# lucidrains/magvit2-pytorch

Hardware: NVIDIA H100
Metric: video-frames/sec tokenize+decode, 17x128x128 bf16 (higher is better)
Workload: dtype bf16

## Files before the change

### magvit2_pytorch_b200/csrc/tc_common.cuh

```cuda
#pragma once
#include "common.cuh"
#include <cuda.h>
#include <mutex>

namespace mv2 {


__device__ __forceinline__ uint32_t smem_u32(const void* p) { return (uint32_t)__cvta_generic_to_shared(p); }

__device__ __forceinline__ void mbar_init(uint32_t bar, uint32_t count) {
  asm volatile("mbarrier.init.shared::cta.b64 [%0], %1;" ::"r"(bar), "r"(count));
}
__device__ __forceinline__ void mbar_expect_tx(uint32_t bar, uint32_t bytes) {
  asm volatile("mbarrier.arrive.expect_tx.shared::cta.b64 _, [%0], %1;" ::"r"(bar), "r"(bytes) : "memory");
}
__device__ __forceinline__ void mbar_wait(uint32_t bar, uint32_t parity) {
  asm volatile(
      "{\n\t"
      ".reg .pred P1;\n\t"
      "WAIT_LOOP:\n\t"
      "mbarrier.try_wait.parity.shared::cta.b64 P1, [%0], %1, 0x989680;\n\t"
      "@P1 bra DONE;\n\t"
      "bra WAIT_LOOP;\n\t"
      "DONE:\n\t"
      "}" ::"r"(bar), "r"(parity) : "memory");
}
__device__ __forceinline__ void fence_barrier_init() { asm volatile("fence.mbarrier_init.release.cluster;" ::: "memory"); }
__device__ __forceinline__ void fence_proxy_async() { asm volatile("fence.proxy.async.shared::cta;" ::: "memory"); }

__device__ __forceinline__ void tma_load_5d(uint32_t dst, const CUtensorMap* map, uint32_t bar, int c0, int c1, int c2,
                                            int c3, int c4) {
  asm volatile(
      "cp.async.bulk.tensor.5d.shared::cluster.global.tile.mbarrier::complete_tx::bytes [%0], [%1, {%3, %4, %5, %6, %7}], [%2];"
      ::"r"(dst), "l"(map), "r"(bar), "r"(c0), "r"(c1), "r"(c2), "r"(c3), "r"(c4) : "memory");
}
__device__ __forceinline__ void tma_load_2d(uint32_t dst, const CUtensorMap* map, uint32_t bar, int c0, int c1) {
  asm volatile(
      "cp.async.bulk.tensor.2d.shared::cluster.global.tile.mbarrier::complete_tx::bytes [%0], [%1, {%3, %4}], [%2];"
      ::"r"(dst), "l"(map), "r"(bar), "r"(c0), "r"(c1) : "memory");
}
__device__ __forceinline__ void tma_load_3d(uint32_t dst, const CUtensorMap* map, uint32_t bar, int c0, int c1, int c2) {
  asm volatile(
      "cp.async.bulk.tensor.3d.shared::cluster.global.tile.mbarrier::complete_tx::bytes [%0], [%1, {%3, %4, %5}], [%2];"
      ::"r"(dst), "l"(map), "r"(bar), "r"(c0), "r"(c1), "r"(c2) : "memory");
}
__device__ __forceinline__ void tma_prefetch_desc(const CUtensorMap* map) {
  asm volatile("prefetch.tensormap [%0];" ::"l"(map) : "memory");
}

__device__ __forceinline__ void wgmma_fence() { asm volatile("wgmma.fence.sync.aligned;" ::: "memory"); }
__device__ __forceinline__ void wgmma_commit() { asm volatile("wgmma.commit_group.sync.aligned;" ::: "memory"); }
__device__ __forceinline__ void wgmma_wait_all() { asm volatile("wgmma.wait_group.sync.aligned 0;" ::: "memory"); }
template <int N> __device__ __forceinline__ void wgmma_bf16(float (&d)[N / 2], uint64_t da, uint64_t db, uint32_t scale_d);
template <> __device__ __forceinline__ void wgmma_bf16<32>(float (&d)[16], uint64_t da, uint64_t db, uint32_t scale_d) {
  asm volatile(
      "{\n\t.reg .pred p;\n\tsetp.ne.b32 p, %18, 0;\n\t"
      "wgmma.mma_async.sync.aligned.m64n32k16.f32.bf16.bf16 {%0, %1, %2, %3, %4, %5, %6, %7, %8, %9, %10, %11, %12, %13, %14, %15}, %16, %17, p, 1, 1, 0, 0;\n\t}"
      : "+f"(d[0]), "+f"(d[1]), "+f"(d[2]), "+f"(d[3]), "+f"(d[4]), "+f"(d[5]), "+f"(d[6]), "+f"(d[7]), "+f"(d[8]), "+f"(d[9]), "+f"(d[10]), "+f"(d[11]), "+f"(d[12]), "+f"(d[13]), "+f"(d[14]), "+f"(d[15])
      : "l"(da), "l"(db), "r"(scale_d));
}
template <> __device__ __forceinline__ void wgmma_bf16<64>(float (&d)[32], uint64_t da, uint64_t db, uint32_t scale_d) {
  asm volatile(
      "{\n\t.reg .pred p;\n\tsetp.ne.b32 p, %34, 0;\n\t"
      "wgmma.mma_async.sync.aligned.m64n64k16.f32.bf16.bf16 {%0, %1, %2, %3, %4, %5, %6, %7, %8, %9, %10, %11, %12, %13, %14, %15, %16, %17, %18, %19, %20, %21, %22, %23, %24, %25, %26, %27, %28, %29, %30, %31}, %32, %33, p, 1, 1, 0, 0;\n\t}"
      : "+f"(d[0]), "+f"(d[1]), "+f"(d[2]), "+f"(d[3]), "+f"(d[4]), "+f"(d[5]), "+f"(d[6]), "+f"(d[7]), "+f"(d[8]), "+f"(d[9]), "+f"(d[10]), "+f"(d[11]), "+f"(d[12]), "+f"(d[13]), "+f"(d[14]), "+f"(d[15]), "+f"(d[16]), "+f"(d[17]), "+f"(d[18]), "+f"(d[19]), "+f"(d[20]), "+f"(d[21]), "+f"(d[22]), "+f"(d[23]), "+f"(d[24]), "+f"(d[25]), "+f"(d[26]), "+f"(d[27]), "+f"(d[28]), "+f"(d[29]), "+f"(d[30]), "+f"(d[31])
      : "l"(da), "l"(db), "r"(scale_d));
}
template <> __device__ __forceinline__ void wgmma_bf16<128>(float (&d)[64], uint64_t da, uint64_t db, uint32_t scale_d) {
  asm volatile(
      "{\n\t.reg .pred p;\n\tsetp.ne.b32 p, %66, 0;\n\t"
      "wgmma.mma_async.sync.aligned.m64n128k16.f32.bf16.bf16 {%0, %1, %2, %3, %4, %5, %6, %7, %8, %9, %10, %11, %12, %13, %14, %15, %16, %17, %18, %19, %20, %21, %22, %23, %24, %25, %26, %27, %28, %29, %30, %31, %32, %33, %34, %35, %36, %37, %38, %39, %40, %41, %42, %43, %44, %45, %46, %47, %48, %49, %50, %51, %52, %53, %54, %55, %56, %57, %58, %59, %60, %61, %62, %63}, %64, %65, p, 1, 1, 0, 0;\n\t}"
      : "+f"(d[0]), "+f"(d[1]), "+f"(d[2]), "+f"(d[3]), "+f"(d[4]), "+f"(d[5]), "+f"(d[6]), "+f"(d[7]), "+f"(d[8]), "+f"(d[9]), "+f"(d[10]), "+f"(d[11]), "+f"(d[12]), "+f"(d[13]), "+f"(d[14]), "+f"(d[15]), "+f"(d[16]), "+f"(d[17]), "+f"(d[18]), "+f"(d[19]), "+f"(d[20]), "+f"(d[21]), "+f"(d[22]), "+f"(d[23]), "+f"(d[24]), "+f"(d[25]), "+f"(d[26]), "+f"(d[27]), "+f"(d[28]), "+f"(d[29]), "+f"(d[30]), "+f"(d[31]), "+f"(d[32]), "+f"(d[33]), "+f"(d[34]), "+f"(d[35]), "+f"(d[36]), "+f"(d[37]), "+f"(d[38]), "+f"(d[39]), "+f"(d[40]), "+f"(d[41]), "+f"(d[42]), "+f"(d[43]), "+f"(d[44]), "+f"(d[45]), "+f"(d[46]), "+f"(d[47]), "+f"(d[48]), "+f"(d[49]), "+f"(d[50]), "+f"(d[51]), "+f"(d[52]), "+f"(d[53]), "+f"(d[54]), "+f"(d[55]), "+f"(d[56]), "+f"(d[57]), "+f"(d[58]), "+f"(d[59]), "+f"(d[60]), "+f"(d[61]), "+f"(d[62]), "+f"(d[63])
      : "l"(da), "l"(db), "r"(scale_d));
}

__host__ __device__ __forceinline__ uint64_t gmma_desc_hi(uint32_t sbo, uint32_t row_bytes) {
  const uint64_t layout = row_bytes == 128 ? 1 : (row_bytes == 64 ? 2 : 3);
  return ((uint64_t)1 << 16) | ((uint64_t)(sbo >> 4) << 32) | (layout << 62);
}
__device__ __forceinline__ uint32_t desc_lo(uint32_t saddr) { return (saddr & 0x3FFFF) >> 4; }

template <int N> __device__ __forceinline__ void stage_acc(const float (&d)[N / 2], float* stg, int t) {
  const int r = 16 * (t >> 5) + ((t & 31) >> 2), c = 2 * (t & 3);
#pragma unroll
  for (int j = 0; j < N / 8; ++j) {
    *reinterpret_cast<float2*>(stg + r * (N + 4) + 8 * j + c) = make_float2(d[4 * j], d[4 * j + 1]);
    *reinterpret_cast<float2*>(stg + (r + 8) * (N + 4) + 8 * j + c) = make_float2(d[4 * j + 2], d[4 * j + 3]);
  }
}
__device__ __forceinline__ void load_row32(const float* src, int ncols, uint32_t (&r)[32]) {
#pragma unroll
  for (int g = 0; g < 8; ++g) {
    if (g * 4 >= ncols) break;
    const float4 v = *reinterpret_cast<const float4*>(src + 4 * g);
    r[4 * g] = __float_as_uint(v.x); r[4 * g + 1] = __float_as_uint(v.y);
    r[4 * g + 2] = __float_as_uint(v.z); r[4 * g + 3] = __float_as_uint(v.w);
  }
}
__device__ __forceinline__ void named_bar_sync(uint32_t id, uint32_t nthreads) {
  asm volatile("bar.sync %0, %1;" ::"r"(id), "r"(nthreads) : "memory");
}
__device__ __forceinline__ void mbar_arrive(uint32_t bar) {
  asm volatile("mbarrier.arrive.shared::cta.b64 _, [%0];" ::"r"(bar) : "memory");
}

__device__ __forceinline__ uint32_t pack_bf16x2(float a, float b) {
  __nv_bfloat162 v = __floats2bfloat162_rn(a, b);
  return *reinterpret_cast<uint32_t*>(&v);
}



struct TcEpi {
  const float* bias;
  const __nv_bfloat16* res;
  __nv_bfloat16* y;
  int act, shuffle, mode;
  int Co;
  int To, Ho, Wo;
  int out_cf;
  const float* oscale;
};

__device__ __forceinline__ void store8_bf16(__nv_bfloat16* dst, const float (&v)[8]) {
  uint4 o;
  o.x = pack_bf16x2(v[0], v[1]); o.y = pack_bf16x2(v[2], v[3]);
  o.z = pack_bf16x2(v[4], v[5]); o.w = pack_bf16x2(v[6], v[7]);
  *reinterpret_cast<uint4*>(dst) = o;
}

enum { EPI_PLAIN = 0, EPI_GEGLU = 1, EPI_SHUFFLE = 2, EPI_RAGGED = 3, EPI_PLAIN_RES = 4, EPI_FUSED_RU = 5, EPI_SHUFFLE_ST = 6,
       EPI_DOWN_SPACE = 7 };

__device__ __forceinline__ float ex2_approx(float x) {
  float y;
  asm("ex2.approx.ftz.f32 %0, %1;" : "=f"(y) : "f"(x));
  return y;
}
__device__ __forceinline__ float rcp_approx(float x) {
  float y;
  asm("rcp.approx.ftz.f32 %0, %1;" : "=f"(y) : "f"(x));
  return y;
}
__device__ __forceinline__ float erf_fast(float x) {
  const float ax = fabsf(x);
  const float t = rcp_approx(fmaf(0.3275911f, ax, 1.f));
  float p = fmaf(1.061405429f, t, -1.453152027f);
  p = fmaf(p, t, 1.421413741f);
  p = fmaf(p, t, -0.284496736f);
  p = fmaf(p, t, 0.254829592f);
  const float e = ex2_approx(-1.4426950408889634f * ax * ax);
  return copysignf(fmaf(-p * t, e, 1.f), x);
}

__device__ __forceinline__ float gelu_fast(float g) {
  const float ag = fabsf(g);
  const float t = rcp_approx(fmaf(0.3275911f * 0.70710678118654752440f, ag, 1.f));
  float p = fmaf(0.5f * 1.061405429f, t, 0.5f * -1.453152027f);
  p = fmaf(p, t, 0.5f * 1.421413741f);
  p = fmaf(p, t, 0.5f * -0.284496736f);
  p = fmaf(p, t, 0.5f * 0.254829592f);
  const float e = ex2_approx((g * g) * (-0.5f * 1.4426950408889634f));
  const float q = (p * t) * e;
  return fmaf(-ag, q, fmaxf(g, 0.f));
}

template <int ACT>
__device__ __forceinline__ float act_ct(float x) {
  if (ACT == MV2_ACT_ELU) {
    const float e = ex2_approx(x * 1.4426950408889634f) - 1.f;
    return x > 0.f ? x : e;
  }
  if (ACT == MV2_ACT_SILU) return x * rcp_approx(1.f + ex2_approx(-1.4426950408889634f * x));
  if (ACT == MV2_ACT_LEAKY_RELU) return x > 0.f ? x : 0.1f * x;
  return x;
}

template <int MODE, int ACT>
__device__ __forceinline__ void epi_chunk32_t(const TcEpi& e, const uint32_t (&r)[32], int ncols, int n, const float* sb,
                                              int b, int to, int ho, int wo, int64_t row_base) {
  if (MODE == EPI_GEGLU) {
    const int I = e.Co >> 1;
    const int64_t pos = (((int64_t)b * e.To + to) * e.Ho + ho) * e.Wo + wo;
#pragma unroll
    for (int g = 0; g < 2; ++g) {
      if (g * 16 >= ncols || n + g * 16 >= e.Co) break;
      float v[8];
#pragma unroll
      for (int q = 0; q < 8; ++q) {
        const float xv = __uint_as_float(r[g * 16 + q]) + sb[g * 16 + q];
        const float gt = __uint_as_float(r[g * 16 + 8 + q]) + sb[g * 16 + 8 + q];
        v[q] = gelu_fast(gt) * xv;
      }
      store8_bf16(e.y + pos * I + ((n + g * 16) >> 1), v);
    }
    return;
  }
  const int cy = MODE == EPI_SHUFFLE ? (e.shuffle == MV2_SHUFFLE_SPACE ? (e.Co >> 2) : (e.Co >> 1)) : e.Co;
  const bool vec_ok = (cy & 7) == 0;
#pragma unroll
  for (int g = 0; g < 4; ++g) {
    const int ng = n + g * 8;
    if (g * 8 >= ncols || ng >= e.Co) break;
    float v[8];
    {
      const float4 b0 = *reinterpret_cast<const float4*>(sb + g * 8), b1 = *reinterpret_cast<const float4*>(sb + g * 8 + 4);
      const float bb[8] = {b0.x, b0.y, b0.z, b0.w, b1.x, b1.y, b1.z, b1.w};
      if (MODE != EPI_SHUFFLE && e.oscale) {
#pragma unroll
        for (int q = 0; q < 8; ++q) {
          const float os = ng + q < e.Co ? e.oscale[(int64_t)b * e.Co + ng + q] : 0.f;
          v[q] = act_ct<ACT>(__uint_as_float(r[g * 8 + q]) * os + bb[q]);
        }
      } else
#pragma unroll
      for (int q = 0; q < 8; ++q) v[q] = act_ct<ACT>(__uint_as_float(r[g * 8 + q]) + bb[q]);
    }
    int64_t off;
    if (MODE == EPI_SHUFFLE) {
      const int qd = ng / cy, c = ng - qd * cy;
      if (e.shuffle == MV2_SHUFFLE_SPACE) {
        const int p1 = qd >> 1, p2 = qd & 1;
        off = ((((int64_t)b * e.To + to) * (2 * e.Ho) + (2 * ho + p1)) * (2 * e.Wo) + (2 * wo + p2)) * cy + c;
      } else {
        off = ((((int64_t)b * (2 * e.To) + (2 * to + qd)) * e.Ho + ho) * e.Wo + wo) * cy + c;
      }
    } else {
      off = row_base + ng;
    }
    const float rscale = e.mode == 2 ? 0.70710678118654752440f : 1.f;
    if (vec_ok && ng + 8 <= e.Co) {
      if (e.res) {
        const uint4 rv = *reinterpret_cast<const uint4*>(e.res + off);
        const __nv_bfloat162* rb = reinterpret_cast<const __nv_bfloat162*>(&rv);
#pragma unroll
        for (int q = 0; q < 4; ++q) {
          const float2 f = __bfloat1622float2(rb[q]);
          v[2 * q] = (v[2 * q] + f.x) * rscale;
          v[2 * q + 1] = (v[2 * q + 1] + f.y) * rscale;
        }
      }
      store8_bf16(e.y + off, v);
    } else {
      if (MODE == EPI_RAGGED && e.out_cf) {
        const int64_t plane = (int64_t)e.Ho * e.Wo;
        const int64_t o0 = ((int64_t)b * e.Co * e.To + to) * plane + (int64_t)ho * e.Wo + wo;
        for (int q = 0; q < 8 && ng + q < e.Co; ++q) e.y[o0 + (int64_t)(ng + q) * e.To * plane] = __float2bfloat16_rn(v[q]);
      } else
      for (int q = 0; q < 8 && ng + q < e.Co; ++q) {
        float x = v[q];
        if (e.res) x = (x + __bfloat162float(e.res[off + q])) * rscale;
        e.y[off + q] = __float2bfloat16_rn(x);
      }
    }
  }
}

template <int ACT>
__device__ __forceinline__ void epi_pack32_t(const uint32_t (&r)[32], const float* sb, uint32_t (&pk)[16]) {
#pragma unroll
  for (int g = 0; g < 8; ++g) {
    const float4 b = *reinterpret_cast<const float4*>(sb + g * 4);
    pk[2 * g] = pack_bf16x2(act_ct<ACT>(__uint_as_float(r[4 * g]) + b.x), act_ct<ACT>(__uint_as_float(r[4 * g + 1]) + b.y));
    pk[2 * g + 1] = pack_bf16x2(act_ct<ACT>(__uint_as_float(r[4 * g + 2]) + b.z), act_ct<ACT>(__uint_as_float(r[4 * g + 3]) + b.w));
  }
}
__device__ __forceinline__ void epi_geglu_pack32(const uint32_t (&r)[32], const float* sb, uint32_t* pk) {
#pragma unroll
  for (int g = 0; g < 2; ++g) {
    float bx[8], bg[8], v[8];
    *reinterpret_cast<float4*>(bx) = *reinterpret_cast<const float4*>(sb + g * 16);
    *reinterpret_cast<float4*>(bx + 4) = *reinterpret_cast<const float4*>(sb + g * 16 + 4);
    *reinterpret_cast<float4*>(bg) = *reinterpret_cast<const float4*>(sb + g * 16 + 8);
    *reinterpret_cast<float4*>(bg + 4) = *reinterpret_cast<const float4*>(sb + g * 16 + 12);
#pragma unroll
    for (int q = 0; q < 8; ++q)
      v[q] = gelu_fast(__uint_as_float(r[g * 16 + 8 + q]) + bg[q]) * (__uint_as_float(r[g * 16 + q]) + bx[q]);
    pk[4 * g] = pack_bf16x2(v[0], v[1]); pk[4 * g + 1] = pack_bf16x2(v[2], v[3]);
    pk[4 * g + 2] = pack_bf16x2(v[4], v[5]); pk[4 * g + 3] = pack_bf16x2(v[6], v[7]);
  }
}
template <int ACT>
__device__ __forceinline__ void epi_act32_t(uint32_t (&r)[32], const float* sb) {
#pragma unroll
  for (int g = 0; g < 8; ++g) {
    const float4 b = *reinterpret_cast<const float4*>(sb + g * 4);
    r[4 * g] = __float_as_uint(act_ct<ACT>(__uint_as_float(r[4 * g]) + b.x));
    r[4 * g + 1] = __float_as_uint(act_ct<ACT>(__uint_as_float(r[4 * g + 1]) + b.y));
    r[4 * g + 2] = __float_as_uint(act_ct<ACT>(__uint_as_float(r[4 * g + 2]) + b.z));
    r[4 * g + 3] = __float_as_uint(act_ct<ACT>(__uint_as_float(r[4 * g + 3]) + b.w));
  }
}
__device__ __forceinline__ void epi_act32(int act, uint32_t (&r)[32], const float* sb) {
  if (act == MV2_ACT_ELU) epi_act32_t<MV2_ACT_ELU>(r, sb);
  else if (act == MV2_ACT_SILU) epi_act32_t<MV2_ACT_SILU>(r, sb);
  else if (act == MV2_ACT_LEAKY_RELU) epi_act32_t<MV2_ACT_LEAKY_RELU>(r, sb);
  else epi_act32_t<MV2_ACT_NONE>(r, sb);
}
__device__ __forceinline__ void epi_pack32(int act, const uint32_t (&r)[32], const float* sb, uint32_t (&pk)[16]) {
  if (act == MV2_ACT_ELU) epi_pack32_t<MV2_ACT_ELU>(r, sb, pk);
  else if (act == MV2_ACT_SILU) epi_pack32_t<MV2_ACT_SILU>(r, sb, pk);
  else if (act == MV2_ACT_LEAKY_RELU) epi_pack32_t<MV2_ACT_LEAKY_RELU>(r, sb, pk);
  else epi_pack32_t<MV2_ACT_NONE>(r, sb, pk);
}

template <int MODE>
__device__ __forceinline__ void epi_chunk32(const TcEpi& e, const uint32_t (&r)[32], int ncols, int n, const float* sb,
                                            int b, int to, int ho, int wo, int64_t row_base) {
  if (MODE == EPI_GEGLU) { epi_chunk32_t<EPI_GEGLU, MV2_ACT_NONE>(e, r, ncols, n, sb, b, to, ho, wo, row_base); return; }
  if (e.act == MV2_ACT_ELU) epi_chunk32_t<MODE, MV2_ACT_ELU>(e, r, ncols, n, sb, b, to, ho, wo, row_base);
  else if (e.act == MV2_ACT_SILU) epi_chunk32_t<MODE, MV2_ACT_SILU>(e, r, ncols, n, sb, b, to, ho, wo, row_base);
  else if (e.act == MV2_ACT_LEAKY_RELU) epi_chunk32_t<MODE, MV2_ACT_LEAKY_RELU>(e, r, ncols, n, sb, b, to, ho, wo, row_base);
  else epi_chunk32_t<MODE, MV2_ACT_NONE>(e, r, ncols, n, sb, b, to, ho, wo, row_base);
}

typedef CUresult (*EncodeTiledFn)(CUtensorMap*, CUtensorMapDataType, cuuint32_t, void*, const cuuint64_t*,
                                  const cuuint64_t*, const cuuint32_t*, const cuuint32_t*, CUtensorMapInterleave,
                                  CUtensorMapSwizzle, CUtensorMapL2promotion, CUtensorMapFloatOOBfill);

static inline EncodeTiledFn get_encode_fn() {
  static EncodeTiledFn fn = nullptr;
  static std::once_flag once;
  std::call_once(once, [] {
    void* f = nullptr;
    cudaDriverEntryPointQueryResult q;
    if (cudaGetDriverEntryPoint("cuTensorMapEncodeTiled", &f, cudaEnableDefault, &q) == cudaSuccess &&
        q == cudaDriverEntryPointSuccess)
      fn = (EncodeTiledFn)f;
  });
  return fn;
}

static inline int pow2_ceil(int v) { int r = 1; while (r < v) r <<= 1; return r; }
static inline int floor_div(int a, int b) { int q = a / b; if ((a % b != 0) && ((a < 0) != (b < 0))) --q; return q; }


}
```

### magvit2_pytorch_b200/csrc/tc_slab.cu

```cuda
#include "common.cuh"
#include "tc_common.cuh"
#include <cuda.h>
#include <algorithm>
#include <mutex>
#include <map>
#include <vector>
#include <string.h>
#include <stdlib.h>

namespace mv2 {

struct alignas(64) SlabParams {
  CUtensorMap amap;
  CUtensorMap wmap;
  CUtensorMap wmap2;
  int kt, kh, kw, pt, ph, pw;
  int st;
  int Ci, kchunks, row_bytes;
  int B, T, H, W, Co;
  int mw, pitch, slab_h, slab_bytes, slab_stride;
  int bn, n_tiles_n, tiles_w, tiles_h, total_tiles;
  int slab_stages, w_stages;
  int tpw;
  int geglu_staged;
  TcEpi epi;
  CUtensorMap w1map;
  const float* bias1;
  const float* se_wk;
  float se_bk;
  float* se_ws;
  CUtensorMap amap_odd;
  int dn_e_off;
  int dn_aoff[6];
  int dn_lower;
  int h_stride;
};

__host__ __device__ __forceinline__ void slab_frame_of(const SlabParams& p, int slot, int& b, int& t) {
  const int ptc = p.pt > 0 ? (p.pt + p.st - 1) / p.st : 0;
  const int n_cheap = ptc < p.T ? ptc : p.T, n_full = p.T - n_cheap;
  const int full_slots = p.B * n_full;
  if (slot < full_slots) { b = slot / n_full; t = n_cheap + slot - b * n_full; }
  else { const int r = slot - full_slots; const int level = r / p.B; b = r - level * p.B; t = n_cheap - 1 - level; }
}
__host__ __device__ __forceinline__ int slab_tile_of_cta(const SlabParams& p, int k, int cta, int grid) {
  const int tile = k * grid + ((k & 1) ? grid - 1 - cta : cta);
  return tile < p.total_tiles ? tile : -1;
}
__device__ __forceinline__ int slab_tile_of(const SlabParams& p, int k) { return slab_tile_of_cta(p, k, blockIdx.x, gridDim.x); }

struct TileCoord { int b, t, h0, w0, n0; };
__host__ __device__ __forceinline__ TileCoord decode_tile(const SlabParams& p, int tile) {
  TileCoord c;
  const int nt = tile % p.n_tiles_n; tile /= p.n_tiles_n;
  const int tw = tile % p.tiles_w; tile /= p.tiles_w;
  const int th = tile % p.tiles_h; tile /= p.tiles_h;
  slab_frame_of(p, tile, c.b, c.t);
  c.h0 = th * 16;
  c.w0 = tw * 8 * p.mw;
  c.n0 = nt * p.bn;
  return c;
}

struct SlabSmem { uint32_t sbias, stage0, lpart, accstg, hbuf, w1buf, end; };
__host__ __device__ __forceinline__ SlabSmem slab_smem_layout(const SlabParams& p, uint32_t bar0, bool fused) {
  SlabSmem m;
  m.sbias = (bar0 + 8 * (2 * p.slab_stages + 2 * p.w_stages + 1) + 15) & ~15u;
  m.stage0 = m.sbias + (uint32_t)(p.n_tiles_n * p.bn) * 4 * (fused ? 3 : 1);
  m.lpart = m.stage0 + (fused ? 0 : 8 * 2048);
  m.accstg = m.lpart + (fused ? 2048 : 0);
  m.hbuf = m.accstg + 2u * p.mw * 64 * (p.bn + 4) * 4;
  if (fused) m.hbuf = (m.hbuf + 1023u) & ~1023u;
  m.w1buf = m.hbuf + (fused ? (uint32_t)p.h_stride : 0);
  m.end = m.w1buf + (fused ? (uint32_t)(p.kchunks * p.bn * p.row_bytes) : 0);
  return m;
}

template <int MODE, int BN>
__global__ void __launch_bounds__(384, 1) tc_slab_kernel(const __grid_constant__ SlabParams p) {
  constexpr int MWMAX = 128 / BN;
  constexpr int NEPI = 8;
  extern __shared__ uint8_t smem_raw[];
  const uint32_t smem_base = (smem_u32(smem_raw) + 1023u) & ~1023u;
  const int warp = threadIdx.x >> 5, lane = threadIdx.x & 31;
  const uint32_t row_bytes = p.row_bytes;
  const uint32_t bk = row_bytes >> 1;
  const uint32_t w_tile = p.bn * row_bytes;
  const uint32_t w_bytes = w_tile * p.tpw;
  const uint32_t slab0 = smem_base;
  const uint32_t wst0 = smem_base + p.slab_stages * p.slab_stride;
  const uint32_t bar0 = wst0 + p.w_stages * w_bytes;
  const uint32_t slab_full = bar0, slab_empty = slab_full + 8 * p.slab_stages;
  const uint32_t w_full = slab_empty + 8 * p.slab_stages, w_empty = w_full + 8 * p.w_stages;
  const uint32_t w1_full = w_empty + 8 * p.w_stages;
  const SlabSmem L = slab_smem_layout(p, bar0, MODE == EPI_FUSED_RU);
  auto gen = [&](uint32_t u) { return smem_raw + (u - smem_u32(smem_raw)); };
  float* sbias = reinterpret_cast<float*>(gen(L.sbias));
  const uint32_t nbias = (uint32_t)(p.n_tiles_n * p.bn);
  const uint32_t stage0 = L.stage0;

  if (threadIdx.x == 0) {
    for (int s = 0; s < p.slab_stages; ++s) { mbar_init(slab_full + 8 * s, 1); mbar_init(slab_empty + 8 * s, 8); }
    for (int s = 0; s < p.w_stages; ++s) { mbar_init(w_full + 8 * s, 1); mbar_init(w_empty + 8 * s, 8); }
    mbar_init(w1_full, 1);
    fence_barrier_init();
  }
  if (warp == 0 && lane == 0) { tma_prefetch_desc(&p.amap); if (MODE == EPI_DOWN_SPACE) tma_prefetch_desc(&p.amap_odd); }
  if (warp == 2 && lane == 0) { tma_prefetch_desc(&p.wmap); tma_prefetch_desc(&p.wmap2); }
  if (MODE == EPI_FUSED_RU && warp == 3 && lane == 0) tma_prefetch_desc(&p.w1map);
  if (warp >= 4) {
    const int nb = p.n_tiles_n * p.bn;
    for (int i = threadIdx.x - 128; i < nb; i += 256) sbias[i] = (p.epi.bias && i < p.Co) ? p.epi.bias[i] : 0.f;
    if (MODE == EPI_FUSED_RU)
      for (int i = threadIdx.x - 128; i < nb; i += 256) {
        sbias[nb + i] = (p.bias1 && i < p.Co) ? p.bias1[i] : 0.f;
        sbias[2 * nb + i] = i < p.Co ? p.se_wk[i] : 0.f;
      }
  }
  __syncthreads();
  pdl_wait();
  pdl_launch_dependents();

  const int taps2d = p.kh * p.kw;

  if (warp == 0) {
    if (MODE == EPI_DOWN_SPACE) {
      if (lane == 0) {
        uint32_t s = 0, ph = 0;
        for (int tk = 0, tile; (tile = slab_tile_of(p, tk)) >= 0; ++tk) {
          const TileCoord c = decode_tile(p, tile);
          for (int kc = 0; kc < p.kchunks; ++kc) {
            mbar_wait(slab_empty + 8 * s, ph ^ 1);
            mbar_expect_tx(slab_full + 8 * s, p.slab_bytes);
            tma_load_5d(slab0 + s * p.slab_stride, &p.amap_odd, slab_full + 8 * s, kc * bk, c.w0 - 1, c.h0 - 1, c.t, c.b);
            tma_load_5d(slab0 + s * p.slab_stride + p.dn_e_off, &p.amap, slab_full + 8 * s, kc * bk, c.w0 - 1, c.h0, c.t, c.b);
            if (++s == (uint32_t)p.slab_stages) { s = 0; ph ^= 1; }
          }
        }
      }
    } else
    if (lane == 0) {
      uint32_t s = 0, ph = 0;
      for (int tk = 0, tile; (tile = slab_tile_of(p, tk)) >= 0; ++tk) {
        const TileCoord c = decode_tile(p, tile);
        const int dt0 = max(0, p.pt - c.t * p.st);
        for (int dt = dt0; dt < p.kt; ++dt)
          for (int kc = 0; kc < p.kchunks; ++kc) {
            mbar_wait(slab_empty + 8 * s, ph ^ 1);
            mbar_expect_tx(slab_full + 8 * s, p.slab_bytes);
            tma_load_5d(slab0 + s * p.slab_stride, &p.amap, slab_full + 8 * s, kc * bk, c.w0 - p.pw, c.h0 - p.ph,
                        c.t * p.st + dt - p.pt, c.b);
            if (++s == (uint32_t)p.slab_stages) { s = 0; ph ^= 1; }
          }
      }
    }
  } else if (warp == 2) {
    if (MODE == EPI_DOWN_SPACE) {
      if (lane == 0) {
        uint32_t s = 0, ph = 0;
        const int C2 = p.Ci;
        for (int tk = 0, tile; (tile = slab_tile_of(p, tk)) >= 0; ++tk) {
          const TileCoord c = decode_tile(p, tile);
          for (int kc = 0; kc < p.kchunks; ++kc)
            for (int tap = kc < p.dn_lower ? 1 : 0; tap < 6; tap += kc < p.dn_lower ? 2 : 1) {
              mbar_wait(w_empty + 8 * s, ph ^ 1);
              mbar_expect_tx(w_full + 8 * s, w_tile);
              tma_load_2d(wst0 + s * w_bytes, &p.wmap2, w_full + 8 * s, tap * C2 + kc * (int)bk, c.n0);
              if (++s == (uint32_t)p.w_stages) { s = 0; ph ^= 1; }
            }
        }
      }
    } else
    if (lane == 0) {
      uint32_t s = 0, ph = 0;
      for (int tk = 0, tile; (tile = slab_tile_of(p, tk)) >= 0; ++tk) {
        const TileCoord c = decode_tile(p, tile);
        const int dt0 = max(0, p.pt - c.t * p.st);
        for (int dt = dt0; dt < p.kt; ++dt)
          for (int kc = 0; kc < p.kchunks; ++kc)
            for (int tp = 0; tp < taps2d; tp += p.tpw) {
              mbar_wait(w_empty + 8 * s, ph ^ 1);
              mbar_expect_tx(w_full + 8 * s, w_bytes);
              if (p.tpw == 1) tma_load_2d(wst0 + s * w_bytes, &p.wmap2, w_full + 8 * s, (dt * taps2d + tp) * p.Ci + kc * bk, c.n0);
              else tma_load_3d(wst0 + s * w_bytes, &p.wmap, w_full + 8 * s, kc * bk, c.n0, dt * taps2d + tp);
              if (++s == (uint32_t)p.w_stages) { s = 0; ph ^= 1; }
            }
      }
    }
  } else if (warp == 3) {
    if (MODE == EPI_FUSED_RU && lane == 0) {
      mbar_expect_tx(w1_full, (uint32_t)p.kchunks * w_tile);
      for (int kc2 = 0; kc2 < p.kchunks; ++kc2) tma_load_2d(L.w1buf + kc2 * w_tile, &p.w1map, w1_full, kc2 * (int)bk, 0);
    }
  } else if (warp >= 4) {
    const int wg = (warp - 4) >> 2, wq = warp & 3, tid = threadIdx.x & 127;
    const int sub = 2 * wg + (wq & 1), half = wq >> 1, ew = sub + 4 * half;
    const int row = sub * 32 + lane;
    const int lh = row >> 3, lw = row & 7;
    float* stg = reinterpret_cast<float*>(gen(L.accstg)) + (size_t)wg * p.mw * 64 * (BN + 4);
    const uint32_t wg_bar = 5 + wg;
    const uint32_t sbo = (uint32_t)p.pitch * row_bytes;
    const uint64_t a_hi = gmma_desc_hi(sbo, row_bytes);
    const uint64_t b_hi = gmma_desc_hi(8 * row_bytes, row_bytes);
    const bool k4 = bk == 64;
    const uint32_t a_row = row_bytes >> 4;
    const uint32_t a_wg = (uint32_t)wg * 8 * (sbo >> 4);
    const uint32_t a_next_dh = (uint32_t)(p.pitch - p.kw + 1) * a_row;
    const uint32_t a_mtile = 8 * a_row;
    const uint32_t w_tile16 = w_tile >> 4, w_stage16 = w_bytes >> 4;
    const uint32_t b_lo0 = desc_lo(wst0);
    uint32_t s_idx = 0, s_par = 0;
    uint32_t w_idx = 0, w_par = 0, b_lo = b_lo0;
    uint32_t ecount = 0;
    if (MODE == EPI_FUSED_RU) mbar_wait(w1_full, 0);
    float acc[MWMAX][BN / 2];
    for (int tk = 0, tile; (tile = slab_tile_of(p, tk)) >= 0; ++tk) {
      const TileCoord c = decode_tile(p, tile);
      uint32_t accum = 0;
      if (MODE == EPI_DOWN_SPACE) {
        for (int kc = 0; kc < p.kchunks; ++kc) {
          mbar_wait(slab_full + 8 * s_idx, s_par);
          const uint32_t a_base = desc_lo(slab0 + s_idx * p.slab_stride) + a_wg;
          const int t0 = kc < p.dn_lower ? 1 : 0, tstep = kc < p.dn_lower ? 2 : 1;
          for (int tap = t0; tap < 6; tap += tstep) {
            mbar_wait(w_full + 8 * w_idx, w_par);
            wgmma_fence();
            const uint64_t bd = b_hi | (uint64_t)b_lo;
#pragma unroll
            for (int j = 0; j < MWMAX; ++j) {
              if (j >= p.mw) break;
              const uint64_t ad = a_hi | (uint64_t)(a_base + (uint32_t)p.dn_aoff[tap] + j * a_mtile);
              wgmma_bf16<BN>(acc[j], ad, bd, accum);
              wgmma_bf16<BN>(acc[j], ad + 2, bd + 2, 1u);
              wgmma_bf16<BN>(acc[j], ad + 4, bd + 4, 1u);
              wgmma_bf16<BN>(acc[j], ad + 6, bd + 6, 1u);
            }
            wgmma_commit();
            wgmma_wait_all();
            __syncwarp();
            if (lane == 0) mbar_arrive(w_empty + 8 * w_idx);
            accum = 1;
            if (++w_idx == (uint32_t)p.w_stages) { w_idx = 0; w_par ^= 1; b_lo = b_lo0; } else { b_lo += w_stage16; }
          }
          if (lane == 0) mbar_arrive(slab_empty + 8 * s_idx);
          if (++s_idx == (uint32_t)p.slab_stages) { s_idx = 0; s_par ^= 1; }
        }
      } else {
        const int dt0 = max(0, p.pt - c.t * p.st);
        for (int dt = dt0; dt < p.kt; ++dt)
          for (int kc = 0; kc < p.kchunks; ++kc) {
            mbar_wait(slab_full + 8 * s_idx, s_par);
            uint32_t a_lo = desc_lo(slab0 + s_idx * p.slab_stride) + a_wg;
            int dw = 0;
            for (int tp0 = 0; tp0 < taps2d; tp0 += p.tpw) {
              mbar_wait(w_full + 8 * w_idx, w_par);
              wgmma_fence();
              uint32_t b_cur = b_lo;
              for (int u = 0; u < p.tpw; ++u) {
                const uint64_t bd = b_hi | (uint64_t)b_cur;
#pragma unroll
                for (int j = 0; j < MWMAX; ++j) {
                  if (j >= p.mw) break;
                  const uint64_t ad = a_hi | (uint64_t)(a_lo + j * a_mtile);
                  wgmma_bf16<BN>(acc[j], ad, bd, accum);
                  wgmma_bf16<BN>(acc[j], ad + 2, bd + 2, 1u);
                  if (k4) {
                    wgmma_bf16<BN>(acc[j], ad + 4, bd + 4, 1u);
                    wgmma_bf16<BN>(acc[j], ad + 6, bd + 6, 1u);
                  }
                }
                accum = 1;
                b_cur += w_tile16;
                if (++dw == p.kw) { dw = 0; a_lo += a_next_dh; } else { a_lo += a_row; }
              }
              wgmma_commit();
              wgmma_wait_all();
              __syncwarp();
              if (lane == 0) mbar_arrive(w_empty + 8 * w_idx);
              if (++w_idx == (uint32_t)p.w_stages) { w_idx = 0; w_par ^= 1; b_lo = b_lo0; } else { b_lo += w_stage16; }
            }
            if (lane == 0) mbar_arrive(slab_empty + 8 * s_idx);
            if (++s_idx == (uint32_t)p.slab_stages) { s_idx = 0; s_par ^= 1; }
          }
      }
      named_bar_sync(wg_bar, 128);
#pragma unroll
      for (int j = 0; j < MWMAX; ++j) {
        if (j >= p.mw) break;
        stage_acc<BN>(acc[j], stg + j * 64 * (BN + 4), tid);
      }
      named_bar_sync(wg_bar, 128);
      const int h = c.h0 + lh;
      if (MODE == EPI_FUSED_RU) {
        const float* sb1 = sbias + nbias;
        const float* swk = sbias + 2 * nbias;
        float* lpart = reinterpret_cast<float*>(gen(L.lpart));
        const int64_t kstride = (int64_t)p.W * p.Co;
        const uint32_t wsw = (lane >> 1) & 3;
        const int rl = lane >> 2, piece = lane & 3;
        const int h20 = c.h0 + sub * 4;
        const int recs_per_frame = p.tiles_h * p.tiles_w * 4;
        float* rec = p.se_ws + ((int64_t)(c.b * p.T + c.t) * recs_per_frame + ((c.h0 >> 4) * p.tiles_w + c.w0 / (8 * p.mw)) * 4 + sub) * (p.Co + 2);
        float run_m = -INFINITY, run_s = 0.f, run_acc[2][8];
#pragma unroll
        for (int q = 0; q < 2; ++q)
#pragma unroll
          for (int i = 0; i < 8; ++i) run_acc[q][i] = 0.f;
        const uint64_t h_hi = gmma_desc_hi(1024, 128);
        const uint32_t h_lo = desc_lo(L.hbuf) + (uint32_t)wg * ((64 * 128) >> 4), w1_lo = desc_lo(L.w1buf);
        for (int j = 0; j < p.mw; ++j) {
          const float* srow = stg + (j * 64 + row - 64 * wg) * (BN + 4);
          const uint32_t stg2 = smem_u32(stg + (j * 64 + (sub & 1) * 32) * (BN + 4)) + (uint32_t)half * 2048;
          const uint32_t wr = stg2 + lane * 64, rd = stg2 + rl * 64;
          const uint32_t hb = L.hbuf + (uint32_t)row * 128;
          for (int c0 = half * 32; c0 < p.bn; c0 += 64) {
            uint32_t r[32], pk[16];
            load_row32(srow + c0, 32, r);
            epi_pack32_t<MV2_ACT_ELU>(r, sbias + c0, pk);
            const uint32_t hrow = hb + (uint32_t)(c0 >> 6) * 16384;
            const uint32_t p0 = (uint32_t)(c0 & 63) >> 3;
#pragma unroll
            for (int g = 0; g < 4; ++g)
              asm volatile("st.shared.v4.b32 [%0], {%1, %2, %3, %4};" ::"r"(hrow + (((p0 + g) ^ ((uint32_t)row & 7u)) << 4)),
                           "r"(pk[4 * g]), "r"(pk[4 * g + 1]), "r"(pk[4 * g + 2]), "r"(pk[4 * g + 3]) : "memory");
          }
          fence_proxy_async();
          named_bar_sync(wg_bar, 128);
          wgmma_fence();
          for (int kc2 = 0; kc2 < p.kchunks; ++kc2) {
            const uint64_t ad = h_hi | (uint64_t)(h_lo + kc2 * (16384 >> 4)), bd = h_hi | (uint64_t)(w1_lo + kc2 * (w_tile >> 4));
            wgmma_bf16<BN>(acc[0], ad, bd, kc2 > 0 ? 1u : 0u);
            wgmma_bf16<BN>(acc[0], ad + 2, bd + 2, 1u);
            wgmma_bf16<BN>(acc[0], ad + 4, bd + 4, 1u);
            wgmma_bf16<BN>(acc[0], ad + 6, bd + 6, 1u);
          }
          wgmma_commit();
          wgmma_wait_all();
          stage_acc<BN>(acc[0], stg + j * 64 * (BN + 4), tid);
          named_bar_sync(wg_bar, 128);
          const int w = c.w0 + 8 * j + lw;
          const bool row_ok = h < p.H && w < p.W;
          uint32_t pk2[2][16];
          float lp = 0.f;
#pragma unroll
          for (int q = 0; q < 2; ++q) {
            const int c0 = half * 32 + 64 * q;
            if (c0 < p.bn) {
              uint32_t r[32];
              load_row32(srow + c0, 32, r);
              epi_pack32_t<MV2_ACT_ELU>(r, sb1 + c0, pk2[q]);
#pragma unroll
              for (int i = 0; i < 16; i += 2) {
                const float4 wv = *reinterpret_cast<const float4*>(swk + c0 + 2 * i);
                lp = fmaf(__uint_as_float(pk2[q][i] << 16), wv.x, lp);
                lp = fmaf(__uint_as_float(pk2[q][i] & 0xffff0000u), wv.y, lp);
                lp = fmaf(__uint_as_float(pk2[q][i + 1] << 16), wv.z, lp);
                lp = fmaf(__uint_as_float(pk2[q][i + 1] & 0xffff0000u), wv.w, lp);
              }
            }
          }
          float* lpb = lpart + (ecount & 1u) * 256;
          ++ecount;
          lpb[ew * 32 + lane] = lp;
          asm volatile("bar.sync %0, 64;" ::"r"(1 + sub) : "memory");
          float lg = lpb[sub * 32 + lane] + lpb[(sub + 4) * 32 + lane] + p.se_bk;
          lg = row_ok ? lg : -INFINITY;
          const float mx = warp_max(lg);
          const float ev = lg > -INFINITY ? ex2_approx((lg - mx) * 1.4426950408889634f) : 0.f;
          const float es = warp_sum(ev);
          float e4[4];
#pragma unroll
          for (int k = 0; k < 4; ++k) e4[k] = __shfl_sync(0xffffffffu, ev, 8 * k + rl);
          const float new_m = fmaxf(run_m, mx);
          const float ca = run_m > -INFINITY ? ex2_approx((run_m - new_m) * 1.4426950408889634f) : 0.f;
          const float cb = mx > -INFINITY ? ex2_approx((mx - new_m) * 1.4426950408889634f) : 0.f;
          run_s = fmaf(run_s, ca, es * cb);
          run_m = new_m;
          const int w2 = c.w0 + 8 * j + rl;
          const int64_t row0 = ((((int64_t)c.b * p.T + c.t) * p.H + h20) * p.W + w2) * p.Co + piece * 8;
          const int kmax = w2 < p.W ? p.H - h20 : 0;
#pragma unroll
          for (int q = 0; q < 2; ++q) {
            const int c0 = half * 32 + 64 * q;
            if (c0 < p.bn) {
#pragma unroll
              for (int g = 0; g < 4; ++g)
                asm volatile("st.shared.v4.b32 [%0], {%1, %2, %3, %4};" ::"r"(wr + ((g ^ wsw) << 4)), "r"(pk2[q][4 * g]),
                             "r"(pk2[q][4 * g + 1]), "r"(pk2[q][4 * g + 2]), "r"(pk2[q][4 * g + 3]) : "memory");
              __syncwarp();
              __nv_bfloat16* yp = p.epi.y + row0 + c0;
              float t[8];
#pragma unroll
              for (int i = 0; i < 8; ++i) t[i] = 0.f;
#pragma unroll
              for (int k = 0; k < 4; ++k) {
                uint4 v;
                asm volatile("ld.shared.v4.b32 {%0, %1, %2, %3}, [%4];" : "=r"(v.x), "=r"(v.y), "=r"(v.z), "=r"(v.w)
                             : "r"(rd + k * 512 + ((piece ^ (((8 * k + rl) >> 1) & 3)) << 4)));
                if (k < kmax) *reinterpret_cast<uint4*>(yp + k * kstride) = v;
                const uint32_t vv[4] = {v.x, v.y, v.z, v.w};
#pragma unroll
                for (int i = 0; i < 4; ++i) {
                  t[2 * i] = fmaf(e4[k], __uint_as_float(vv[i] << 16), t[2 * i]);
                  t[2 * i + 1] = fmaf(e4[k], __uint_as_float(vv[i] & 0xffff0000u), t[2 * i + 1]);
                }
              }
              __syncwarp();
#pragma unroll
              for (int i = 0; i < 8; ++i) {
                t[i] += __shfl_xor_sync(0xffffffffu, t[i], 4);
                t[i] += __shfl_xor_sync(0xffffffffu, t[i], 8);
                t[i] += __shfl_xor_sync(0xffffffffu, t[i], 16);
              }
#pragma unroll
              for (int i = 0; i < 8; ++i) run_acc[q][i] = fmaf(run_acc[q][i], ca, t[i] * cb);
            }
          }
        }
        if (half == 0 && lane == 0) { rec[0] = run_m; rec[1] = run_s; }
        if (rl == 0) {
#pragma unroll
          for (int q = 0; q < 2; ++q) {
            const int c0 = half * 32 + 64 * q;
            if (c0 < p.bn) {
              float2* dst = reinterpret_cast<float2*>(rec + 2 + c0 + piece * 8);
              dst[0] = make_float2(run_acc[q][0], run_acc[q][1]); dst[1] = make_float2(run_acc[q][2], run_acc[q][3]);
              dst[2] = make_float2(run_acc[q][4], run_acc[q][5]); dst[3] = make_float2(run_acc[q][6], run_acc[q][7]);
            }
          }
        }
      } else
      for (int j = 0; j < p.mw; ++j) {
        const int w = c.w0 + 8 * j + lw;
        const bool row_ok = h < p.H && w < p.W;
        const float* srow = stg + (j * 64 + row - 64 * wg) * (BN + 4);
        const int64_t row_base = ((((int64_t)c.b * p.T + c.t) * p.H + h) * p.W + w) * p.Co;
        if (MODE == EPI_PLAIN || MODE == EPI_PLAIN_RES || MODE == EPI_SHUFFLE_ST || MODE == EPI_DOWN_SPACE) {
          const uint32_t stg = stage0 + (uint32_t)ew * 2048;
          const uint32_t wr = stg + lane * 64, wsw = (lane >> 1) & 3;
          const int rl = lane >> 2, piece = lane & 3;
          const int w2 = c.w0 + 8 * j + rl;
          const uint32_t rd = stg + rl * 64;
          const int h20 = c.h0 + sub * 4;
          const int64_t row0 = ((((int64_t)c.b * p.T + c.t) * p.H + h20) * p.W + w2) * p.Co + c.n0 + piece * 8;
          const int64_t kstride = (int64_t)p.W * p.Co;
          const int kmax = w2 < p.W ? p.H - h20 : 0;
          for (int c0 = ((j + half) & 1) * 32; c0 < p.bn; c0 += 64) {
            uint32_t r[32], pk[16];
            uint4 rv[4];
            if (MODE == EPI_PLAIN_RES) {
              const __nv_bfloat16* rr = p.epi.res + row_base + c.n0 + c0;
#pragma unroll
              for (int g = 0; g < 4; ++g)
                rv[g] = (row_ok && c.n0 + c0 + g * 8 < p.Co && c0 + g * 8 < p.bn) ? *reinterpret_cast<const uint4*>(rr + g * 8) : make_uint4(0, 0, 0, 0);
            }
            load_row32(srow + c0, 32, r);
            if ((MODE == EPI_PLAIN || MODE == EPI_PLAIN_RES) && p.epi.oscale) {
              const float* os = p.epi.oscale + (int64_t)c.b * p.Co + c.n0 + c0;
#pragma unroll
              for (int i = 0; i < 32; ++i) r[i] = __float_as_uint(__uint_as_float(r[i]) * (c.n0 + c0 + i < p.Co ? os[i] : 0.f));
            }
            if (MODE == EPI_PLAIN_RES) {
              epi_act32(p.epi.act, r, sbias + c.n0 + c0);
              const float rs = p.epi.mode == 2 ? 0.70710678118654752440f : 1.f;
#pragma unroll
              for (int g = 0; g < 4; ++g) {
                const uint32_t w4[4] = {rv[g].x, rv[g].y, rv[g].z, rv[g].w};
#pragma unroll
                for (int q = 0; q < 4; ++q)
                  pk[4 * g + q] = pack_bf16x2((__uint_as_float(r[8 * g + 2 * q]) + __uint_as_float(w4[q] << 16)) * rs,
                                              (__uint_as_float(r[8 * g + 2 * q + 1]) + __uint_as_float(w4[q] & 0xffff0000u)) * rs);
              }
            } else
            epi_pack32(p.epi.act, r, sbias + c.n0 + c0, pk);
#pragma unroll
            for (int g = 0; g < 4; ++g)
              asm volatile("st.shared.v4.b32 [%0], {%1, %2, %3, %4};" ::"r"(wr + ((g ^ wsw) << 4)), "r"(pk[4 * g]),
                           "r"(pk[4 * g + 1]), "r"(pk[4 * g + 2]), "r"(pk[4 * g + 3]) : "memory");
            __syncwarp();
            const bool col_ok = c.n0 + c0 + piece * 8 < p.Co && c0 + piece * 8 < p.bn;
            const int klim = col_ok ? kmax : 0;
            __nv_bfloat16* yp;
            int64_t ks;
            if (MODE == EPI_SHUFFLE_ST) {
              const int n = c.n0 + c0;
              if (p.epi.shuffle == MV2_SHUFFLE_SPACE) {
                const int cy = p.Co >> 2, qd = n / cy, cb = n - qd * cy;
                yp = p.epi.y + ((((int64_t)c.b * p.T + c.t) * (2 * p.H) + (2 * h20 + (qd >> 1))) * (2 * p.W) + (2 * w2 + (qd & 1))) * cy + cb + piece * 8;
                ks = (int64_t)4 * p.W * cy;
              } else {
                const int cy = p.Co >> 1, qd = n / cy, cb = n - qd * cy;
                yp = p.epi.y + ((((int64_t)c.b * (2 * p.T) + (2 * c.t + qd)) * p.H + h20) * p.W + w2) * cy + cb + piece * 8;
                ks = (int64_t)p.W * cy;
              }
            } else {
              yp = p.epi.y + row0 + c0;
              ks = kstride;
            }
#pragma unroll
            for (int k = 0; k < 4; ++k) {
              uint4 v;
              asm volatile("ld.shared.v4.b32 {%0, %1, %2, %3}, [%4];" : "=r"(v.x), "=r"(v.y), "=r"(v.z), "=r"(v.w)
                           : "r"(rd + k * 512 + ((piece ^ (((8 * k + rl) >> 1) & 3)) << 4)));
              if (k < klim) *reinterpret_cast<uint4*>(yp + k * ks) = v;
            }
            __syncwarp();
          }
        } else if (MODE == EPI_GEGLU && p.geglu_staged) {
          const uint32_t stg = stage0 + (uint32_t)ew * 2048;
          const uint32_t wr = stg + lane * 64, wsw = (lane >> 1) & 3;
          const int rl = lane >> 2, piece = lane & 3;
          const int w2 = c.w0 + 8 * j + rl;
          const uint32_t rd = stg + rl * 64;
          const int h20 = c.h0 + sub * 4;
          const int I = p.Co >> 1;
          const int64_t row0 = ((((int64_t)c.b * p.T + c.t) * p.H + h20) * p.W + w2) * I + (c.n0 >> 1) + piece * 8;
          const int64_t ks = (int64_t)p.W * I;
          const int kmax = w2 < p.W ? p.H - h20 : 0;
          const int nch = p.bn >> 6;
          for (int c0 = 0; c0 < p.bn; c0 += 64) {
            if (((j * nch + (c0 >> 6)) & (NEPI / 4 - 1)) != half) continue;
            uint32_t r0[32], r1[32], pk[16];
            load_row32(srow + c0, 32, r0);
            load_row32(srow + c0 + 32, 32, r1);
            epi_geglu_pack32(r0, sbias + c.n0 + c0, pk);
            epi_geglu_pack32(r1, sbias + c.n0 + c0 + 32, pk + 8);
#pragma unroll
            for (int g = 0; g < 4; ++g)
              asm volatile("st.shared.v4.b32 [%0], {%1, %2, %3, %4};" ::"r"(wr + ((g ^ wsw) << 4)), "r"(pk[4 * g]),
                           "r"(pk[4 * g + 1]), "r"(pk[4 * g + 2]), "r"(pk[4 * g + 3]) : "memory");
            __syncwarp();
            const bool col_ok = c.n0 + c0 + piece * 16 < p.Co && c0 + piece * 16 < p.bn;
            const int klim = col_ok ? kmax : 0;
            __nv_bfloat16* yp = p.epi.y + row0 + (c0 >> 1);
#pragma unroll
            for (int k = 0; k < 4; ++k) {
              uint4 v;
              asm volatile("ld.shared.v4.b32 {%0, %1, %2, %3}, [%4];" : "=r"(v.x), "=r"(v.y), "=r"(v.z), "=r"(v.w)
                           : "r"(rd + k * 512 + ((piece ^ (((8 * k + rl) >> 1) & 3)) << 4)));
              if (k < klim) *reinterpret_cast<uint4*>(yp + k * ks) = v;
            }
            __syncwarp();
          }
        } else {
          for (int c0 = ((j + half) & 1) * 32; c0 < p.bn; c0 += 64) {
            uint32_t r[32];
            load_row32(srow + c0, 32, r);
            if (row_ok) epi_chunk32<MODE>(p.epi, r, min(32, p.bn - c0), c.n0 + c0, sbias + c.n0 + c0, c.b, c.t, h, w, row_base);
          }
        }
      }
    }
  }
}

}

using namespace mv2;

#define MV2_SLAB_BN(M) {tc_slab_kernel<M, 32>, tc_slab_kernel<M, 64>, tc_slab_kernel<M, 128>}
static void (*const g_slab_kernels[8][3])(SlabParams) = {
    MV2_SLAB_BN(EPI_PLAIN), MV2_SLAB_BN(EPI_GEGLU), MV2_SLAB_BN(EPI_SHUFFLE), MV2_SLAB_BN(EPI_RAGGED),
    MV2_SLAB_BN(EPI_PLAIN_RES), MV2_SLAB_BN(EPI_FUSED_RU), MV2_SLAB_BN(EPI_SHUFFLE_ST), MV2_SLAB_BN(EPI_DOWN_SPACE)};
#undef MV2_SLAB_BN
static void (*slab_kernel_for(int mode, int bn))(SlabParams) { return g_slab_kernels[mode][bn == 32 ? 0 : (bn == 64 ? 1 : 2)]; }
static cudaError_t slab_set_smem_attr() {
  static PerDeviceOnce once;
  return once.run([] {
    cudaError_t e = cudaSuccess;
    for (auto& row : g_slab_kernels)
      for (auto k : row)
        if (e == cudaSuccess) e = cudaFuncSetAttribute(k, cudaFuncAttributeMaxDynamicSharedMemorySize, 227 * 1024);
    return e;
  });
}


extern "C" int mv2_tc_slab_supported(const mv2_tc_conv_args* a) {
  if (!a) return 0;
  if (a->sh != 1 || a->sw != 1) return 0;
  if (a->st != 1) {
    if (a->st != 2 || a->out_layout != 0 || a->epi_mode != 0 || a->shuffle != MV2_SHUFFLE_NONE) return 0;
    if (a->To != (a->Ti + a->pt - a->kt) / a->st + 1 || a->To < 1) return 0;
  }
  if (a->Ci % 32 != 0 || a->Co > 4096) return 0;
  if (a->oscale && (a->epi_mode != 0 || a->shuffle != MV2_SHUFFLE_NONE)) return 0;
  if (a->epi_mode == 1 && (a->Co % 64 != 0 || a->shuffle != MV2_SHUFFLE_NONE || a->res)) return 0;
// ... 400 lines not shown
```

Baseline: 4503.

## Keep one wgmma group in flight and specialize mainloop on tile width

Restructures the consumer mainloop so each tap issues its own wgmma group and waits with wait_group<1> instead of waiting for all groups. Release of weight and slab stages to the producer is deferred by one group when enough pipeline stages exist. The loop is also templated on compile-time tile width and K depth, which removes runtime breaks in the unrolled loops. This overlaps tensor-core execution with barrier waits and issue, at the cost of holding buffers longer, more commit/wait overhead per tap, and more code from the template instantiations.

```diff
diff --git a/magvit2_pytorch_b200/csrc/tc_common.cuh b/magvit2_pytorch_b200/csrc/tc_common.cuh
--- a/magvit2_pytorch_b200/csrc/tc_common.cuh
+++ b/magvit2_pytorch_b200/csrc/tc_common.cuh
@@ -51,6 +51,11 @@
 __device__ __forceinline__ void wgmma_fence() { asm volatile("wgmma.fence.sync.aligned;" ::: "memory"); }
 __device__ __forceinline__ void wgmma_commit() { asm volatile("wgmma.commit_group.sync.aligned;" ::: "memory"); }
 __device__ __forceinline__ void wgmma_wait_all() { asm volatile("wgmma.wait_group.sync.aligned 0;" ::: "memory"); }
+template <int N> __device__ __forceinline__ void wgmma_wait() { asm volatile("wgmma.wait_group.sync.aligned %0;" ::"n"(N) : "memory"); }
+template <int N> __device__ __forceinline__ void wgmma_fence_operand(float (&d)[N]) {
+#pragma unroll
+  for (int i = 0; i < N; ++i) asm volatile("" : "+f"(d[i])::"memory");
+}
 template <int N> __device__ __forceinline__ void wgmma_bf16(float (&d)[N / 2], uint64_t da, uint64_t db, uint32_t scale_d);
 template <> __device__ __forceinline__ void wgmma_bf16<32>(float (&d)[16], uint64_t da, uint64_t db, uint32_t scale_d) {
   asm volatile(
diff --git a/magvit2_pytorch_b200/csrc/tc_slab.cu b/magvit2_pytorch_b200/csrc/tc_slab.cu
--- a/magvit2_pytorch_b200/csrc/tc_slab.cu
+++ b/magvit2_pytorch_b200/csrc/tc_slab.cu
@@ -7,6 +7,7 @@
 #include <vector>
 #include <string.h>
 #include <stdlib.h>
+#include <type_traits>
 
 namespace mv2 {
 
@@ -214,8 +215,56 @@
     uint32_t ecount = 0;
     if (MODE == EPI_FUSED_RU) mbar_wait(w1_full, 0);
     float acc[MWMAX][BN / 2];
-    for (int tk = 0, tile; (tile = slab_tile_of(p, tk)) >= 0; ++tk) {
-      const TileCoord c = decode_tile(p, tile);
+    uint32_t held = (p.w_stages > 2 && (p.slab_stages > 2 || p.kh * p.kw > p.tpw)) ? 4u : 0u;
+    auto deep = [&]() { return (held & 4u) != 0; };
+    auto release = [&]() {
+      __syncwarp();
+      if (lane == 0) {
+        if (held & 1u) mbar_arrive(w_empty + 8 * (w_idx == 0 ? p.w_stages - 1 : w_idx - 1));
+        if (held & 2u) mbar_arrive(slab_empty + 8 * (s_idx == 0 ? p.slab_stages - 1 : s_idx - 1));
+      }
+      held &= 4u;
+    };
+    auto mainloop = [&](const TileCoord& c, auto mw_c, auto k4_c) {
+      constexpr int MW = decltype(mw_c)::value;
+      constexpr bool K4 = decltype(k4_c)::value;
+      auto fence_acc = [&]() {
+#pragma unroll
+        for (int j = 0; j < MW; ++j) wgmma_fence_operand(acc[j]);
+      };
+      auto tap_mma = [&](uint32_t a_lo, uint64_t bd, uint32_t accum) {
+#pragma unroll
+        for (int j = 0; j < MW; ++j) {
+          const uint64_t ad = a_hi | (uint64_t)(a_lo + j * a_mtile);
+          wgmma_bf16<BN>(acc[j], ad, bd, accum);
+          wgmma_bf16<BN>(acc[j], ad + 2, bd + 2, 1u);
+          if (K4) {
+            wgmma_bf16<BN>(acc[j], ad + 4, bd + 4, 1u);
+            wgmma_bf16<BN>(acc[j], ad + 6, bd + 6, 1u);
+          }
+        }
+      };
+      auto tap_group = [&](uint32_t a_lo, uint64_t bd, uint32_t accum) {
+        fence_acc();
+        wgmma_fence();
+        tap_mma(a_lo, bd, accum);
+        wgmma_commit();
+        fence_acc();
+        if (deep()) wgmma_wait<1>();
+        else wgmma_wait<0>();
+        fence_acc();
+        release();
+      };
+      auto next_w = [&]() {
+        held |= 1u;
+        if (++w_idx == (uint32_t)p.w_stages) { w_idx = 0; w_par ^= 1; b_lo = b_lo0; } else { b_lo += w_stage16; }
+        if (!deep()) release();
+      };
+      auto next_s = [&]() {
+        held |= 2u;
+        if (++s_idx == (uint32_t)p.slab_stages) { s_idx = 0; s_par ^= 1; }
+        if (!deep()) release();
+      };
       uint32_t accum = 0;
       if (MODE == EPI_DOWN_SPACE) {
         for (int kc = 0; kc < p.kchunks; ++kc) {
@@ -224,26 +273,11 @@
           const int t0 = kc < p.dn_lower ? 1 : 0, tstep = kc < p.dn_lower ? 2 : 1;
           for (int tap = t0; tap < 6; tap += tstep) {
             mbar_wait(w_full + 8 * w_idx, w_par);
-            wgmma_fence();
-            const uint64_t bd = b_hi | (uint64_t)b_lo;
-#pragma unroll
-            for (int j = 0; j < MWMAX; ++j) {
-              if (j >= p.mw) break;
-              const uint64_t ad = a_hi | (uint64_t)(a_base + (uint32_t)p.dn_aoff[tap] + j * a_mtile);
-              wgmma_bf16<BN>(acc[j], ad, bd, accum);
-              wgmma_bf16<BN>(acc[j], ad + 2, bd + 2, 1u);
-              wgmma_bf16<BN>(acc[j], ad + 4, bd + 4, 1u);
-              wgmma_bf16<BN>(acc[j], ad + 6, bd + 6, 1u);
-            }
-            wgmma_commit();
-            wgmma_wait_all();
-            __syncwarp();
-            if (lane == 0) mbar_arrive(w_empty + 8 * w_idx);
+            tap_group(a_base + (uint32_t)p.dn_aoff[tap], b_hi | (uint64_t)b_lo, accum);
             accum = 1;
-            if (++w_idx == (uint32_t)p.w_stages) { w_idx = 0; w_par ^= 1; b_lo = b_lo0; } else { b_lo += w_stage16; }
-          }
-          if (lane == 0) mbar_arrive(slab_empty + 8 * s_idx);
-          if (++s_idx == (uint32_t)p.slab_stages) { s_idx = 0; s_par ^= 1; }
+            next_w();
+          }
+          next_s();
         }
       } else {
         const int dt0 = max(0, p.pt - c.t * p.st);
@@ -254,35 +288,32 @@
             int dw = 0;
             for (int tp0 = 0; tp0 < taps2d; tp0 += p.tpw) {
               mbar_wait(w_full + 8 * w_idx, w_par);
-              wgmma_fence();
               uint32_t b_cur = b_lo;
               for (int u = 0; u < p.tpw; ++u) {
-                const uint64_t bd = b_hi | (uint64_t)b_cur;
-#pragma unroll
-                for (int j = 0; j < MWMAX; ++j) {
-                  if (j >= p.mw) break;
-                  const uint64_t ad = a_hi | (uint64_t)(a_lo + j * a_mtile);
-                  wgmma_bf16<BN>(acc[j], ad, bd, accum);
-                  wgmma_bf16<BN>(acc[j], ad + 2, bd + 2, 1u);
-                  if (k4) {
-                    wgmma_bf16<BN>(acc[j], ad + 4, bd + 4, 1u);
-                    wgmma_bf16<BN>(acc[j], ad + 6, bd + 6, 1u);
-                  }
-                }
+                tap_group(a_lo, b_hi | (uint64_t)b_cur, accum);
                 accum = 1;
                 b_cur += w_tile16;
                 if (++dw == p.kw) { dw = 0; a_lo += a_next_dh; } else { a_lo += a_row; }
               }
-              wgmma_commit();
-              wgmma_wait_all();
-              __syncwarp();
-              if (lane == 0) mbar_arrive(w_empty + 8 * w_idx);
-              if (++w_idx == (uint32_t)p.w_stages) { w_idx = 0; w_par ^= 1; b_lo = b_lo0; } else { b_lo += w_stage16; }
+              next_w();
             }
-            if (lane == 0) mbar_arrive(slab_empty + 8 * s_idx);
-            if (++s_idx == (uint32_t)p.slab_stages) { s_idx = 0; s_par ^= 1; }
+            next_s();
           }
       }
+      wgmma_wait<0>();
+      fence_acc();
+      release();
+    };
+    for (int tk = 0, tile; (tile = slab_tile_of(p, tk)) >= 0; ++tk) {
+      const TileCoord c = decode_tile(p, tile);
+      auto by_width = [&](auto mw_c) {
+        if constexpr (MODE == EPI_FUSED_RU || MODE == EPI_DOWN_SPACE) mainloop(c, mw_c, std::true_type{});
+        else if (k4) mainloop(c, mw_c, std::true_type{});
+        else mainloop(c, mw_c, std::false_type{});
+      };
+      if (MWMAX >= 4 && p.mw == 4) by_width(std::integral_constant<int, (MWMAX >= 4 ? 4 : 1)>{});
+      else if (MWMAX >= 2 && p.mw == 2) by_width(std::integral_constant<int, (MWMAX >= 2 ? 2 : 1)>{});
+      else by_width(std::integral_constant<int, 1>{});
       named_bar_sync(wg_bar, 128);
 #pragma unroll
       for (int j = 0; j < MWMAX; ++j) {
```

After: 4574 (median of 6 runs). +1.6%, better.
